# 7IBBE77S/nbodysim

Hardware: AMD Instinct MI355X
Metric: particle-pair interactions/sec at N=262,144 (direct O(N^2) softened gravity + kick/drift step) (higher is better)
Workload: dtype f32

## Files before the change

include/nbody.h:

```cpp
#ifndef NBODY_H
#define NBODY_H

#include <stddef.h>
#include <stdint.h>

#ifdef __cplusplus
extern "C" {
#endif
#pragma GCC visibility push(default)

#define NB_ABI_VERSION 8

typedef struct nb_vec2 {
    float x, y;
    float _pad[2];
} nb_vec2;

#define NB_Z(v) ((v)._pad[0])

typedef struct nb_body {
    nb_vec2 pos;
    nb_vec2 vel;
    nb_vec2 acc;
    float   mass;
// ... 328 lines not shown
    int64_t  r_base;
    uint32_t diag, group;
} nb_sym_item;

typedef struct nb_sym_info {
    uint32_t struct_size;
    int32_t  enabled;
    uint32_t chunks_per_item;
    uint32_t items, items_local, items_cross, items_late;
    uint32_t tiles, rows_s, segments, cus;
    uint64_t units_local, units_cross, units_late;
    uint64_t cross_units_total;
    uint64_t slab_s_bytes, slab_r_bytes;
    uint64_t coverage_entries;
    uint32_t tile_particles;
    uint32_t _reserved0;
} nb_sym_info;
int nb_sym_plan_info(const nb_sim *s, nb_sym_info *out);

int nb_device_count(void);

const char *nb_last_error(void);
int nb_last_error_code(void);

int nb_abi_version(void);

#pragma GCC visibility pop
#ifdef __cplusplus
}
#endif
#endif
// ... 1 lines not shown
```

nbodysim_amd/_lib.py:

```python
from __future__ import annotations

import ctypes as C
import os
from pathlib import Path

import numpy as np

PKG_DIR = Path(__file__).resolve().parent
LIB_PATH = PKG_DIR / "libnbody_hip.so"

NB_ABI_VERSION = 8

NB_OK, NB_EINVAL, NB_ENODEVICE, NB_EHIP, NB_ENOMEM, NB_EIO, NB_EFORMAT, NB_ESTATE = 0, -1, -2, -3, -4, -5, -6, -7
NB_FP32, NB_FP64 = 0, 1
NB_RSQRT_EXACT, NB_RSQRT_QUAKE = 0, 1
NB_SUM_TILED, NB_SUM_SEQUENTIAL = 0, 1
NB_EXTRA_VCLAMP, NB_EXTRA_BOUNDARY, NB_EXTRA_COLLIDE = 1, 2, 4
NB_INTEGRATOR_KICK_DRIFT, NB_INTEGRATOR_KDK, NB_INTEGRATOR_DKD, NB_INTEGRATOR_FR4 = 0, 1, 2, 3
NB_INTEGRATOR_HERMITE4 = 5
NB_FORCE_DIRECT, NB_FORCE_TREE = 0, 1
NB_POS_CURRENT, NB_POS_NEXT = 0, 1
NB_SHARD_NONE, NB_SHARD_ALLGATHER, NB_SHARD_SYMMETRIC, NB_SHARD_ALLREDUCE = 0, 1, 2, 3
NB_FLAG_NO_SYMMETRY, NB_FLAG_NO_UNIFORM_MASS, NB_FLAG_NO_GUIDED_TAIL, NB_FLAG_SHARD_ALLREDUCE, NB_FLAG_SHARD_SINGLE, NB_FLAG_MASS_SCALING = 1, 2, 4, 8, 16, 32
NB_FLAG_STATIC_ITEMS = 256
# ... 125 lines not shown
        ("items_local", C.c_uint32),
        ("items_cross", C.c_uint32),
        ("items_late", C.c_uint32),
        ("tiles", C.c_uint32),
        ("rows_s", C.c_uint32),
        ("segments", C.c_uint32),
        ("cus", C.c_uint32),
        ("units_local", C.c_uint64),
        ("units_cross", C.c_uint64),
        ("units_late", C.c_uint64),
        ("cross_units_total", C.c_uint64),
        ("slab_s_bytes", C.c_uint64),
        ("slab_r_bytes", C.c_uint64),
        ("coverage_entries", C.c_uint64),
        ("tile_particles", C.c_uint32),
        ("_reserved0", C.c_uint32),
    ]

    def as_dict(self) -> dict:
        return {k: int(getattr(self, k)) for k, _ in self._fields_ if k != "struct_size" and not k.startswith("_")}


class nb_view(C.Structure):

    _fields_ = [
        ("struct_size", C.c_uint32),
        ("width", C.c_uint32),
        ("height", C.c_uint32),
        ("center_x", C.c_float),
        ("center_y", C.c_float),
        ("scale", C.c_float),
# ... 206 lines not shown
```

nbodysim_amd/csrc/nb_capi.hip:

```cpp
#include "nb_sim.hip.h"

extern "C" int nb_device_count(void)
{
    int n = 0;
    if (hipGetDeviceCount(&n) != hipSuccess) { (void)hipGetLastError(); return 0; }
    return n;
}

static uint32_t even_slices(uint32_t jn, uint32_t want)
{
    const uint32_t tiles = (jn + TJ - 1) / TJ;
    if (want < 1) want = 1;
    if (want > tiles) want = tiles;
    const uint32_t per = (tiles + want - 1) / want;
    return (tiles + per - 1) / per;
}

static ForceJob plan_job(const nb_sim *s, uint32_t jb, uint32_t je, uint32_t slab0,
                         uint32_t gap_begin = 0xffffffffu, uint32_t gap_len = 0)
{
    ForceJob j{jb, je, 0, slab0, 1, 0, gap_begin, gap_len};
    const uint32_t ic = (uint32_t)s->i_count;
    if (je <= jb) return j;
    const uint32_t jn = je - jb;
// ... 120 lines not shown
static bool sym_uses_pairs(const nb_sim *s)
{
    if (!s->sym_pairs) return false;
    return s->dims3 ? s->uniform_mass || s->p.sym_chunk_pairs > 0 : !s->mass_scaled;
}

static SymTuning tuning_of(const nb_params &p, bool fp64, int cus, uint32_t world, bool sharded, size_t n)
{
    SymTuning t;
    t.forced_L = p.sym_chunks_per_item > 0 ? (uint32_t)p.sym_chunks_per_item : 0u;
    t.late_units = sharded ? late_units_for(p, fp64, cus, world) : 0u;
    t.wg_per_cu = sharded ? 24u : 0u;
    t.late_chunks = fp64 ? 1u : 2u;
    t.even_chunks = want_pairs(p, n);
    t.sb = sym_tile_of(p, n);
    t.guided_tail = !(p.flags & NB_FLAG_NO_GUIDED_TAIL);
    if (p.sym_tail[0] > 0.0f || p.sym_tail[1] > 0.0f || p.sym_tail[2] > 0.0f)
        { for (int k = 0; k < 3; ++k) t.tail_at[k] = (double)p.sym_tail[k]; t.tail_given = true; }
    return t;
}

static void fill_sym_info(const SymPlan &pl, uint32_t n, uint32_t world, int cus, size_t esz, bool enabled, nb_sym_info *out)
{
    const uint32_t sz = out->struct_size;
    memset(out, 0, sizeof *out);
    out->struct_size = sz;
    out->enabled = enabled ? 1 : 0;
    out->chunks_per_item = pl.L;
    out->items = (uint32_t)pl.items.size();
    out->items_local = pl.n_local; out->items_cross = pl.n_cross; out->items_late = pl.n_late;
    out->tiles = pl.tiles;
    out->rows_s = pl.rowbase.empty() ? 0u : pl.rowbase[pl.tiles];
    out->segments = (uint32_t)pl.segs.size();
    out->cus = (uint32_t)cus;
    out->units_local = pl.units_local; out->units_cross = pl.units_cross; out->units_late = pl.units_late;
    sym_units(n, world, nullptr, &out->cross_units_total, pl.sb);
    out->slab_s_bytes = (uint64_t)out->rows_s * pl.sb * esz;
    out->tile_particles = pl.sb;
    out->slab_r_bytes = pl.slab_r_elems * esz;
    out->coverage_entries = pl.cov_main.size() + pl.cov_late.size();
}

#ifdef NB_TEST_HOOKS
extern "C" int nb_debug_sym_plan(size_t n, int cus, int rank, int world, const nb_params *tuning,
                                 nb_sym_item *items_out, size_t cap, nb_sym_info *info)
{
    static_assert(sizeof(nb_sym_item) == sizeof(SymItem) && offsetof(nb_sym_item, r_base) == offsetof(SymItem, r_base) &&
                  offsetof(nb_sym_item, group) == offsetof(SymItem, group), "nb_sym_item mirrors SymItem");
    if (n == 0 || n > 0x7fffff00u || cus < 1 || world < 1 || rank < 0 || rank >= world ||
        (world > 1 && (n % ((size_t)world * SYM_SB)) != 0)) return nb_fail(NB_EINVAL, "nb_debug_sym_plan: bad arguments");
    if (tuning && tuning->struct_size != sizeof(nb_params)) return nb_fail(NB_EINVAL, "nb_debug_sym_plan: tuning->struct_size");
    if (info && info->struct_size != sizeof(nb_sym_info)) return nb_fail(NB_EINVAL, "nb_debug_sym_plan: info->struct_size");
    nb_params p;
    if (tuning) p = *tuning; else nb_params_default(&p);
    p.shard_rank = rank; p.shard_world = world;
// ... 114 lines not shown
    const uint32_t n = (uint32_t)s->n;
    const bool sharded = s->path == StepPath::SYM_SHARDED, split = s->path != StepPath::SYM;
    const uint32_t world = split ? (uint32_t)s->p.shard_world : 1u;
    const uint32_t rank = split ? (uint32_t)s->p.shard_rank : 0u;
    SymPlan pl;
    build_sym_plan(n, (uint32_t)s->cus, rank, world, tuning_of(s->p, s->fp64, s->cus, world, sharded, s->n), pl);
    s->sym_pairs = want_pairs(s->p, s->n);
    const uint32_t tiles = pl.tiles, row = pl.rowbase[tiles];
    s->sym_info.struct_size = (uint32_t)sizeof(nb_sym_info);
    fill_sym_info(pl, n, world, s->cus, s->esz, true, &s->sym_info);
    s->sym_items_local = pl.n_local; s->sym_items_cross = pl.n_cross; s->sym_items_late = pl.n_late;
    s->sym_items = (uint32_t)pl.items.size(); s->sym_tiles = tiles; s->sym_rows = row; s->sym_L = pl.L;
    s->sym_sb = pl.sb; s->sym_sb_shift = pl.sb == SYM_SB_WS ? 9u : 11u;
    std::vector<uint32_t> bounds(3 * (size_t)tiles);
    for (uint32_t g = 0; g < tiles; ++g) { bounds[g] = pl.rowbase[g]; bounds[tiles + g] = pl.rowmid[g]; bounds[2 * (size_t)tiles + g] = pl.rowbase[g + 1]; }
    std::vector<uint32_t> cbegin(pl.cov_main_begin);
    cbegin.insert(cbegin.end(), pl.cov_late_begin.begin(), pl.cov_late_begin.end());
    std::vector<SymCov> cov(pl.cov_main);
    cov.insert(cov.end(), pl.cov_late.begin(), pl.cov_late.end());
    s->sym_cov_late_off = (uint32_t)pl.cov_main.size();
    HIPCHK(s->pool.alloc(s->sym_items_dev, pl.items.size()));
    HIPCHK(s->pool.alloc(s->sym_rowbase_dev, bounds.size()));
    HIPCHK(s->pool.alloc(s->sym_cov_begin_dev, cbegin.size()));
    HIPCHK(s->pool.alloc(s->sym_cov_dev, cov.size() ? cov.size() : 1));
    HIPCHK(s->pool.alloc(s->sym_slab_s, (size_t)(row ? row : 1) * pl.sb * s->esz));
    HIPCHK(s->pool.alloc(s->sym_slab_r, (size_t)(pl.slab_r_elems ? pl.slab_r_elems : 1) * s->esz));
    int rc;
    if ((rc = copy_h2d(s, s->sym_items_dev, pl.items.data(), pl.items.size() * sizeof(SymItem)))) return rc;
    if ((rc = copy_h2d(s, s->sym_rowbase_dev, bounds.data(), bounds.size() * sizeof(uint32_t)))) return rc;
    if ((rc = copy_h2d(s, s->sym_cov_begin_dev, cbegin.data(), cbegin.size() * sizeof(uint32_t)))) return rc;
    if ((rc = copy_h2d(s, s->sym_cov_dev, cov.data(), cov.size() * sizeof(SymCov)))) return rc;
    HIPCHK(s->pool.alloc(s->sym_ticket, 3 * 128 / sizeof(uint32_t)));
    HIPCHK(hipMemsetAsync(s->sym_ticket, 0, 3 * 128, s->stream));
    s->aux_local = sharded && (s->p.sym_aux_stream ? s->p.sym_aux_stream > 0 : s->sym_items_local <= 4u * (uint32_t)s->cus);
    if (s->aux_local || s->sym_items_late) {
        HIPCHK(hipStreamCreateWithFlags(&s->aux, hipStreamNonBlocking));
        HIPCHK(hipEventCreateWithFlags(&s->ev_fork, hipEventDisableTiming));
        HIPCHK(hipEventCreateWithFlags(&s->ev_join, hipEventDisableTiming));
        HIPCHK(hipEventCreateWithFlags(&s->ev_late, hipEventDisableTiming));
    }
    if (split) {
// ... 1314 lines not shown
```

nbodysim_amd/csrc/nb_fuzz.cpp:

```cpp
#include <unistd.h>

#include <algorithm>
#include <cstdio>
#include <cstdlib>
#include <cstring>
#include <random>
#include <string>
#include <vector>

#include "nb_mem.h"
#include "nb_plan.h"
#include "nb_sched.h"
#include "nbody.h"

using namespace nbk;

#define REQUIRE(cond, ...)                                                        \
    do {                                                                          \
        if (!(cond)) {                                                            \
            std::fprintf(stderr, "FAIL %s:%d: %s | ", __FILE__, __LINE__, #cond); \
            std::fprintf(stderr, __VA_ARGS__);                                    \
            std::fprintf(stderr, "\n");                                           \
            std::exit(1);                                                         \
        }                                                                         \
    } while (0)

static void check_plan_case(uint32_t n, uint32_t world, uint32_t cus, const SymTuning &tune)
{
    const uint32_t sb = tune.sb;
    const uint32_t tiles = (n + sb - 1) / sb, chunks = (n + SYM_CH - 1) / SYM_CH, cpt = sb / SYM_CH;
    std::vector<uint8_t> cover((size_t)tiles * chunks, 0);
    uint64_t cross_seen = 0, cross_total = 0;
    sym_units(n, world, nullptr, &cross_total, sb);
    for (uint32_t rank = 0; rank < world; ++rank) {
        SymPlan pl;
        build_sym_plan(n, cus, rank, world, tune, pl);
        REQUIRE(pl.tiles == tiles && pl.sb == sb && pl.items.size() == (size_t)pl.n_local + pl.n_cross + pl.n_late, "n=%u world=%u", n, world);
        REQUIRE(pl.slab_r_elems <= sym_slab_r_bound(n, world, sb), "bound n=%u world=%u: %llu > %llu", n, world,
                (unsigned long long)pl.slab_r_elems, (unsigned long long)sym_slab_r_bound(n, world, sb));
        if (!tune.forced_L) REQUIRE(pl.L % tune.quantum() == 0, "L = %u is not a multiple of the kernel's chunk quantum %u", pl.L, tune.quantum());
        std::vector<uint8_t> row_used(pl.rowbase[tiles], 0);
        std::vector<std::pair<int64_t, int64_t>> ranges;
        for (const SymItem &it : pl.items) {
            REQUIRE(it.tile < tiles && it.cnt >= 1 && it.c0 + it.cnt <= chunks, "item out of range n=%u", n);
            REQUIRE(it.s_row < row_used.size() && !row_used[it.s_row], "stationary row reused n=%u", n);
            row_used[it.s_row] = 1;
            const uint32_t lo_row = it.group == 2 ? pl.rowmid[it.tile] : pl.rowbase[it.tile];
            const uint32_t hi_row = it.group == 2 ? pl.rowbase[it.tile + 1] : pl.rowmid[it.tile];
            REQUIRE(it.s_row >= lo_row && it.s_row < hi_row, "row outside its tile's range");
            if (it.diag) REQUIRE(it.c0 >= it.tile * cpt && it.c0 + it.cnt <= std::min((it.tile + 1) * cpt, chunks), "diag chunks");
            else {
                REQUIRE(it.c0 >= (it.tile + 1) * cpt, "symmetric item meets its own tile");
                const int64_t lo = it.r_base + (int64_t)it.c0 * SYM_CH;
                const int64_t hi = it.r_base + (int64_t)std::min<uint64_t>((uint64_t)(it.c0 + it.cnt) * SYM_CH, n);
                REQUIRE(lo >= 0 && hi <= (int64_t)pl.slab_r_elems && lo < hi, "travelling range outside the slab");
                ranges.push_back({lo, hi});
            }
            if (it.group == 1) cross_seen += it.cnt;
            for (uint32_t c = it.c0; c < it.c0 + it.cnt; ++c) {
                REQUIRE(cover[(size_t)it.tile * chunks + c] == 0, "unit (%u,%u) covered twice, n=%u world=%u", it.tile, c, n, world);
                cover[(size_t)it.tile * chunks + c] = 1;
            }
        }
        std::sort(ranges.begin(), ranges.end());
        int64_t end = 0;
        for (auto &r : ranges) { REQUIRE(r.first == end || r.first == end + 1, "travelling ranges overlap or leave a hole"); end = r.second; }
// ... 2 lines not shown
        auto check_cov = [&](size_t s0, size_t s1, const std::vector<uint32_t> &begin, const std::vector<SymCov> &cov) {
            REQUIRE(begin.size() == (size_t)tiles + 1 && begin[tiles] == cov.size(), "coverage CSR shape");
            uint64_t want = 0, got = 0;
            for (size_t s = s0; s < s1; ++s) want += pl.segs[s].hi - pl.segs[s].lo;
            for (uint32_t t = 0; t < tiles; ++t)
                for (uint32_t i = begin[t]; i < begin[t + 1]; ++i) {
                    const uint32_t a = std::max(cov[i].lo, t * sb), b = std::min<uint64_t>(cov[i].hi, (uint64_t)(t + 1) * sb);
                    REQUIRE(a < b, "coverage entry does not meet its tile");
                    REQUIRE(cov[i].base + (int64_t)a >= 0 && cov[i].base + (int64_t)b <= (int64_t)pl.slab_r_elems, "coverage outside the slab");
                    got += b - a;
                }
            REQUIRE(want == got, "coverage lists miss particles: %llu vs %llu", (unsigned long long)want, (unsigned long long)got);
        };
        check_cov(0, pl.nsegs_main, pl.cov_main_begin, pl.cov_main);
        check_cov(pl.nsegs_main, pl.segs.size(), pl.cov_late_begin, pl.cov_late);
    }
    for (uint32_t t = 0; t < tiles; ++t)
        for (uint32_t c = 0; c < chunks; ++c)
            REQUIRE(cover[(size_t)t * chunks + c] == (c >= t * cpt ? 1 : 0), "unit (%u,%u) cover %d, n=%u world=%u", t, c,
                    cover[(size_t)t * chunks + c], n, world);
    REQUIRE(cross_seen == cross_total, "cross units %llu != %llu", (unsigned long long)cross_seen, (unsigned long long)cross_total);
}

static void fuzz_planner(int cases, std::mt19937 &rng)
{
    for (int k = 0; k < cases; ++k) {
        const uint32_t world = 1 + rng() % 8;
        uint32_t n;
        if (world == 1) n = 1 + rng() % 200000;
        else n = world * SYM_SB * (2 + rng() % 12);
        const uint32_t cus = 1 + rng() % 304;
        SymTuning t;
        if (rng() % 3 == 0) t.forced_L = 1 + rng() % 70;
        if (world > 1 && rng() % 2) t.late_units = rng() % 3000;
        t.late_chunks = 1 + rng() % 3;
        t.guided_tail = rng() % 4 != 0;
        t.even_chunks = rng() % 2 != 0;
        if (rng() % 2) t.sb = SYM_SB_WS;
        if (rng() % 5 == 0) t.wg_per_cu = 8 + rng() % 32;
        if (rng() % 4 == 0) { t.tail_at[0] = 0.3; t.tail_at[1] = 0.6; t.tail_at[2] = 0.9; }
        check_plan_case(n, world, cus, t);
    }
    check_plan_case(262144, 8, 256, SymTuning{});
    { SymTuning e; e.even_chunks = true; e.late_units = 1400; check_plan_case(262144, 8, 256, e); check_plan_case(262144, 1, 256, e); check_plan_case(70001, 1, 256, e); }
    { SymTuning w; w.sb = SYM_SB_WS; check_plan_case(25000, 1, 256, w); check_plan_case(65536, 1, 256, w); check_plan_case(1, 1, 256, w); check_plan_case(513, 1, 2, w);
      w.even_chunks = true; check_plan_case(65536, 1, 256, w); check_plan_case(70001, 1, 256, w); check_plan_case(262144, 8, 256, w); }
    check_plan_case(1, 1, 256, SymTuning{});
    check_plan_case(2048, 1, 256, SymTuning{});
    check_plan_case(2049, 1, 1, SymTuning{});
}

static void write_raw(const std::string &path, const void *data, size_t bytes)
{
    FILE *f = std::fopen(path.c_str(), "wb");
    REQUIRE(f, "cannot create %s", path.c_str());
    REQUIRE(std::fwrite(data, 1, bytes, f) == bytes, "short write");
    std::fclose(f);
}

static void fuzz_host(const std::string &dir, std::mt19937 &rng)
{
    const std::string path = dir + "/fuzz.nbd";
    for (size_t n : {(size_t)1, (size_t)2, (size_t)4097, (size_t)10000}) {
        std::vector<nb_body> b(n), back(n);
// ... 258 lines not shown
```

nbodysim_amd/csrc/nb_kernels.hip.h:

```cpp
#pragma once
#include <hip/hip_runtime.h>
#include <stdint.h>
#include <type_traits>

#include "nb_plan.h"

namespace nbk {

typedef float v2f __attribute__((ext_vector_type(2)));
typedef float v4f __attribute__((ext_vector_type(4)));

constexpr int BLOCK = 256;
constexpr int TJ = 256;

enum { RSQ_EXACT = 0, RSQ_QUAKE = 1 };

constexpr float PAD_XY = 1.0e18f;

template <typename real> struct vec2_of;
template <> struct vec2_of<float> { typedef float2 type; };
template <> struct vec2_of<double> { typedef double2 type; };

template <typename real> struct vec4_of;
template <> struct vec4_of<float> { typedef float4 type; };
// ... 414 lines not shown
#define NB_SYM_UNROLL2 2
#endif
constexpr int SYM_P = NB_SYM_P;
constexpr int SYM_UNROLL = NB_SYM_UNROLL;
constexpr int SYM_UNROLL2 = NB_SYM_UNROLL2;
constexpr uint32_t SYM_WT = 64 * 2 * SYM_P;
static_assert(4 * SYM_WT == SYM_SB, "block-tile of the planner (nb_plan.h) = 4 waves x 64 lanes x 2 SYM_P particles");

__device__ __forceinline__ float lane_rot(float v, int addr)
{
    return __builtin_bit_cast(float, __builtin_amdgcn_ds_bpermute(addr, __builtin_bit_cast(int, v)));
}

enum { MM_UNIFORM = 0, MM_GENERAL = 1, MM_SCALED = 2 };

template <int RSQ, int MM, bool DIAG, bool WS = false, bool WT = false, typename L = Layout<float, false>>
__device__ __forceinline__
void sym_chunks(const typename L::vec *__restrict__ pos, const float *__restrict__ mass, const float *__restrict__ sigma,
                typename L::vec *__restrict__ slab_r_row, uint32_t n, uint32_t c0, uint32_t cnt,
                const v2f (&xi)[SYM_P], const v2f (&yi)[SYM_P], const v2f (&zi)[SYM_P], const v2f (&mi)[SYM_P],
                v2f (&ax)[SYM_P], v2f (&ay)[SYM_P], v2f (&az)[SYM_P], float eps2, float um_mass, typename L::vec (*red)[4][64])
{
    constexpr bool UM = MM == MM_UNIFORM, MS = MM == MM_SCALED;
    const uint32_t t = threadIdx.x, lane = t & 63u, w = t >> 6;
    const int addr = (int)(((lane + 1u) & 63u) * 4u);
    const v2f e2 = {eps2, eps2};

    float xq = PAD_XY, yq = PAD_XY, zq = PAD_XY, mq = MS ? -1.0f : 0.f, eq = eps2;
    auto fetch = [&](uint32_t j, float &x, float &y, float &z, float &m, float &e) {
        x = PAD_XY; y = PAD_XY; z = PAD_XY; m = MS ? -1.0f : 0.f; e = eps2;
        if (j < n) {
// ... 70 lines not shown
            if constexpr (L::dims3) zq = zr;
            if constexpr (!UM) mq = mr;
            if constexpr (MS) eq = er;
            if constexpr (!DIAG) {
                aqx.x = lane_rot(aqx.x, addr); aqx.y = lane_rot(aqx.y, addr);
                aqy.x = lane_rot(aqy.x, addr); aqy.y = lane_rot(aqy.y, addr);
                if constexpr (L::dims3) { aqz.x = lane_rot(aqz.x, addr); aqz.y = lane_rot(aqz.y, addr); }
            }
        }
        if constexpr (!DIAG) {
            typename L::vec r;
            if constexpr (L::dims3) r = make_float4(aqx.x + aqx.y, aqy.x + aqy.y, aqz.x + aqz.y, 0.f);
            else r = make_float2(aqx.x + aqx.y, aqy.x + aqy.y);
            if constexpr (UM) { r.x *= um_mass; r.y *= um_mass; if constexpr (L::dims3) r.z *= um_mass; }
            if constexpr (MS) { const float s2 = mq * mq; r.x *= s2; r.y *= s2; }
            if constexpr (WS) {
                const uint32_t j = (c0 + c) * SYM_CH + lane;
                if (j < n) store8<WT>(&slab_r_row[j], r);
            } else {
                typename L::vec (*rb)[64] = red[c & 1u];
                rb[w][lane] = r;
                __syncthreads();
                if (w == 0) {
                    const uint32_t j = (c0 + c) * SYM_CH + lane;
                    typename L::vec a = rb[0][lane];
#pragma unroll
                    for (int k = 1; k < 4; ++k) { a.x += rb[k][lane].x; a.y += rb[k][lane].y; if constexpr (L::dims3) a.z += rb[k][lane].z; }
                    if (j < n) { if constexpr (L::dims3) slab_r_row[j] = a; else store8<WT>(&slab_r_row[j], a); }
                }
            }
        }
        xq = xn; yq = yn;
        if constexpr (L::dims3) zq = zn;
        if constexpr (!UM) mq = mn;
        if constexpr (MS) eq = en;
    }
}

template <int RSQ, int MM, bool DIAG, bool WS = false, bool WT = false, typename L = Layout<float, false>>
__device__ __forceinline__
void sym_chunks2(const typename L::vec *__restrict__ pos, const float *__restrict__ mass,
                 typename L::vec *__restrict__ slab_r_row, uint32_t n, uint32_t c0, uint32_t cnt,
                 const v2f (&xi)[SYM_P], const v2f (&yi)[SYM_P], const v2f (&zi)[SYM_P], const v2f (&mi)[SYM_P],
                 v2f (&ax)[SYM_P], v2f (&ay)[SYM_P], v2f (&az)[SYM_P], float eps2, float um_mass, float4 (*red)[4][64])
{
    static_assert(MM != MM_SCALED, "the mass-scaled body keeps the one-chunk form");
    constexpr bool UM = MM == MM_UNIFORM;
    const uint32_t t = threadIdx.x, lane = t & 63u, w = t >> 6;
    const int addr = (int)(((lane + 1u) & 63u) * 4u);
    const v2f e2 = {eps2, eps2};
    v2f bx[2 * SYM_P], by[2 * SYM_P], bz[2 * SYM_P];
#pragma unroll
    for (int k = 0; k < 2 * SYM_P; ++k) { bx[k] = (v2f){0.f, 0.f}; by[k] = (v2f){0.f, 0.f}; bz[k] = (v2f){0.f, 0.f}; }

// ... 68 lines not shown
                    }
                }
            }
            xq = xr; yq = yr;
            if constexpr (L::dims3) zq = zr;
            if constexpr (!UM) mq = mr;
            if constexpr (!DIAG) {
                aqx = (v2f){lane_rot(aqx.x, addr), lane_rot(aqx.y, addr)};
                aqy = (v2f){lane_rot(aqy.x, addr), lane_rot(aqy.y, addr)};
                if constexpr (L::dims3) aqz = (v2f){lane_rot(aqz.x, addr), lane_rot(aqz.y, addr)};
            }
        }
        if constexpr (!DIAG && L::dims3) {
            float4 r0 = make_float4(aqx.x, aqy.x, aqz.x, 0.f), r1 = make_float4(aqx.y, aqy.y, aqz.y, 0.f);
            if constexpr (UM) { r0.x *= um_mass; r0.y *= um_mass; r0.z *= um_mass; r1.x *= um_mass; r1.y *= um_mass; r1.z *= um_mass; }
            float4 (*rb)[4][64] = red + 2u * ((c >> 1) & 1u);
            rb[0][w][lane] = r0;
            rb[1][w][lane] = r1;
            __syncthreads();
            if (w < 2 && c + w < cnt) {
                const uint32_t j = (c0 + c + w) * SYM_CH + lane;
                float4 a = rb[w][0][lane];
#pragma unroll
                for (int k = 1; k < 4; ++k) { a.x += rb[w][k][lane].x; a.y += rb[w][k][lane].y; a.z += rb[w][k][lane].z; }
                if (j < n) slab_r_row[j] = a;
            }
        } else if constexpr (!DIAG) {
            float4 r = make_float4(aqx.x, aqy.x, aqx.y, aqy.y);
            if constexpr (UM) { r.x *= um_mass; r.y *= um_mass; r.z *= um_mass; r.w *= um_mass; }
            if constexpr (WS) {
                const uint32_t j0 = (c0 + c) * SYM_CH + lane, j1 = j0 + SYM_CH;
                if (j0 < n) store8<WT>(&slab_r_row[j0], make_float2(r.x, r.y));
                if (c + 1 < cnt && j1 < n) store8<WT>(&slab_r_row[j1], make_float2(r.z, r.w));
            } else {
                float4 (*rb)[64] = red[(c >> 1) & 1u];
                rb[w][lane] = r;
                __syncthreads();
                if (w < 2 && c + w < cnt) {
                    const uint32_t j = (c0 + c + w) * SYM_CH + lane;
                    float2 a = w ? make_float2(rb[0][lane].z, rb[0][lane].w) : make_float2(rb[0][lane].x, rb[0][lane].y);
#pragma unroll
                    for (int k = 1; k < 4; ++k) {
                        a.x += w ? rb[k][lane].z : rb[k][lane].x;
                        a.y += w ? rb[k][lane].w : rb[k][lane].y;
                    }
// ... 46 lines not shown
            if (g0 < n) p0 = pos[g0];
            if (g1 < n) p1 = pos[g1];
            xi[p] = (v2f){p0.x, p1.x}; yi[p] = (v2f){p0.y, p1.y}; zi[p] = (v2f){p0.z, p1.z}; mi[p] = (v2f){p0.w, p1.w};
            az[p] = (v2f){0.f, 0.f};
        } else {
            float2 p0 = make_float2(PAD_XY, PAD_XY), p1 = p0;
            float m0 = 0.f, m1 = 0.f;
            if (g0 < n) { p0 = pos[g0]; if constexpr (!UM) m0 = mass[g0]; }
            if (g1 < n) { p1 = pos[g1]; if constexpr (!UM) m1 = mass[g1]; }
            xi[p] = (v2f){p0.x, p1.x}; yi[p] = (v2f){p0.y, p1.y}; mi[p] = (v2f){m0, m1};
        }
        ax[p] = (v2f){0.f, 0.f}; ay[p] = (v2f){0.f, 0.f};
    }
    NB_STAMP(1);
    typename L::vec *__restrict__ rrow = slab_r + it.r_base;
    if constexpr (PAIRS) {
        if (diag) sym_chunks2<RSQ, MM, true, WS, WT, L>(pos, mass, rrow, n, it.c0, it.cnt, xi, yi, zi, mi, ax, ay, az, eps2, um_mass, red2);
        else      sym_chunks2<RSQ, MM, false, WS, WT, L>(pos, mass, rrow, n, it.c0, it.cnt, xi, yi, zi, mi, ax, ay, az, eps2, um_mass, red2);
    } else {
        if (diag) sym_chunks<RSQ, MM, true, WS, WT, L>(pos, mass, sigma, rrow, n, it.c0, it.cnt, xi, yi, zi, mi, ax, ay, az, eps2, um_mass, red);
        else      sym_chunks<RSQ, MM, false, WS, WT, L>(pos, mass, sigma, rrow, n, it.c0, it.cnt, xi, yi, zi, mi, ax, ay, az, eps2, um_mass, red);
    }

    NB_STAMP(2);
    typename L::vec *__restrict__ out = slab_s + (size_t)s_row * SB;
    if constexpr (L::dims3) {
#pragma unroll
        for (int p = 0; p < SYM_P; ++p) {
            if constexpr (UM) { ax[p] *= um_mass; ay[p] *= um_mass; az[p] *= um_mass; }
            out[li[p]] = make_float4(ax[p].x, ay[p].x, az[p].x, 0.f);
            out[li[p] + 1] = make_float4(ax[p].y, ay[p].y, az[p].y, 0.f);
        }
    } else if constexpr (WS) {
#pragma unroll
        for (int p = 0; p < SYM_P; ++p) red4[w * SYM_P + p][lane] = make_float4(ax[p].x, ay[p].x, ax[p].y, ay[p].y);
        __syncthreads();
// ... 25 lines not shown

template <int RSQ, int MM, bool PAIRS = false, bool WS = false>
__global__ __launch_bounds__(BLOCK, NB_SYM_WAVES)
void force_sym_f32(const float2 *__restrict__ pos, const float *__restrict__ mass, const float *__restrict__ sigma,
                   const SymItem *__restrict__ items,
                   float2 *__restrict__ slab_s, float2 *__restrict__ slab_r,
                   uint32_t n, float eps2, float um_mass, uint32_t *ticket, uint32_t first_wave, uint32_t ticket_base)
{
#ifndef NB_SYM_WT
#define NB_SYM_WT true
#endif
    force_sym_f32_body<RSQ, MM, PAIRS, WS, NB_SYM_WT>(pos, mass, sigma, items[sym_item_index(ticket, first_wave, ticket_base)], slab_s, slab_r, n, eps2, um_mass);
}

template <int RSQ, bool UM, bool PAIRS = false>
__global__ __launch_bounds__(BLOCK, UM && !PAIRS ? 5 : 1)
void force_sym3_f32(const float4 *__restrict__ pos, const SymItem *__restrict__ items,
                    float4 *__restrict__ slab_s, float4 *__restrict__ slab_r, uint32_t n, float eps2, float um_mass,
                    uint32_t *ticket, uint32_t first_wave, uint32_t ticket_base)
{
    force_sym_f32_body<RSQ, UM ? MM_UNIFORM : MM_GENERAL, PAIRS, false, false, Layout<float, true>>(
        pos, nullptr, nullptr, items[sym_item_index(ticket, first_wave, ticket_base)], slab_s, slab_r, n, eps2, um_mass);
}

__global__ __launch_bounds__(BLOCK)
void mass_sigma(const float *__restrict__ mass, float *__restrict__ sigma, uint32_t n)
{
    const uint32_t i = blockIdx.x * BLOCK + threadIdx.x;
    if (i < n) sigma[i] = 1.0f / sqrtf(mass[i]);
}

// ... 709 lines not shown
```

nbodysim_amd/csrc/nb_plan.cpp:

```cpp
#include "nb_plan.h"

#include <cmath>

namespace nbk {

namespace {
struct Geometry {
    uint32_t n, world, sb, tiles, chunks, cpt, tpb;
    Geometry(uint32_t n_, uint32_t world_, uint32_t sb_) : n(n_), world(world_ ? world_ : 1), sb(sb_ ? sb_ : SYM_SB)
    {
        tiles = (n + sb - 1) / sb;
        chunks = (n + SYM_CH - 1) / SYM_CH;
        cpt = sb / SYM_CH;
        tpb = world > 1 ? (n / world) / sb : tiles;
        if (tpb == 0) tpb = 1;
    }
    uint32_t block_of(uint32_t I) const { return I / tpb; }
    uint32_t block_end_chunk(uint32_t I) const
    {
        const uint64_t e = (uint64_t)(I / tpb + 1) * tpb * cpt;
        return (world > 1 && e < chunks) ? (uint32_t)e : chunks;
    }
    uint32_t diag_end(uint32_t I) const { return (I + 1) * cpt < chunks ? (I + 1) * cpt : chunks; }
};
// ... 8 lines not shown
        const uint32_t be = g.block_end_chunk(I);
        const uint32_t b = g.world > 1 ? g.block_of(I) : 0;
        if (b < g.world) local_of[b] += be - g.diag_end(I);
        cross += g.chunks - be;
    }
    for (uint64_t v : local_of) if (v > local_max) local_max = v;
    if (local_sym_units) *local_sym_units = local_max;
    if (cross_total) *cross_total = cross;
}

uint64_t sym_slab_r_bound(uint32_t n, uint32_t world, uint32_t sb)
{
    uint64_t local = 0, cross = 0;
    sym_units(n, world, &local, &cross, sb);
    const uint64_t w = world ? world : 1;
    return (local + (cross + w - 1) / w + (uint64_t)(n / SYM_CH) + (sb ? sb : SYM_SB) / SYM_CH) * SYM_CH;
}

void build_sym_plan(uint32_t n, uint32_t cus, uint32_t rank, uint32_t world, const SymTuning &tune, SymPlan &pl)
{
    const Geometry g(n, world, tune.sb);
    world = g.world;
    const uint32_t tiles = g.tiles, chunks = g.chunks;
    if (cus < 1) cus = 1;

    uint64_t local = 0, cross_total = 0;
    for (uint32_t I = 0; I < tiles; ++I) {
        const uint32_t be = g.block_end_chunk(I);
        if (g.block_of(I) == rank || world == 1) local += be - I * g.cpt;
        cross_total += chunks - be;
    }
// ... 124 lines not shown
        next_cross[I] = row; row += cross_rows_of[I];
        pl.rowmid[I] = row;
        next_late[I] = row; row += late_rows_of[I];
        if (lhi[I] > llo[I]) add_seg(I, llo[I], lhi[I], 0u, base_local);
        if (chi[I] > clo[I]) add_seg(I, clo[I], chi[I], 1u, base_cross);
    }
    pl.rowbase[tiles] = row;
    pl.nsegs_main = (uint32_t)pl.segs.size();
    for (uint32_t I = 0; I < tiles; ++I)
        if (thi[I] > tlo[I]) add_seg(I, tlo[I], thi[I], 2u, base_late);
    pl.slab_r_elems = off;
    pl.units_local = pl.units_cross = pl.units_late = 0;
    for (auto &it : local_items) { it.s_row = next_local[it.tile]++; it.r_base = base_local[it.tile]; it.group = 0u; pl.units_local += it.cnt; }
    for (auto &it : cross_items) { it.s_row = next_cross[it.tile]++; it.r_base = base_cross[it.tile]; it.group = 1u; pl.units_cross += it.cnt; }
    for (auto &it : late_items)  { it.s_row = next_late[it.tile]++;  it.r_base = base_late[it.tile];  it.group = 2u; pl.units_late += it.cnt; }
    pl.n_local = (uint32_t)local_items.size();
    pl.n_cross = (uint32_t)cross_items.size();
    pl.n_late = (uint32_t)late_items.size();
    pl.items = std::move(local_items);
    pl.items.insert(pl.items.end(), cross_items.begin(), cross_items.end());
    pl.items.insert(pl.items.end(), late_items.begin(), late_items.end());
    pl.L = L;
    pl.tiles = tiles;
    pl.sb = g.sb;

    auto build_cov = [&](size_t s0, size_t s1, std::vector<uint32_t> &begin, std::vector<SymCov> &cov) {
        begin.assign((size_t)tiles + 1, 0);
        for (size_t s = s0; s < s1; ++s) {
            const SymSeg &sg = pl.segs[s];
            for (uint32_t t = sg.lo / g.sb; t <= (sg.hi - 1) / g.sb; ++t) ++begin[t + 1];
        }
        for (uint32_t t = 0; t < tiles; ++t) begin[t + 1] += begin[t];
        cov.assign(begin[tiles], SymCov{0, 0u, 0u});
        std::vector<uint32_t> fill(begin.begin(), begin.end() - 1);
        for (size_t s = s0; s < s1; ++s) {
            const SymSeg &sg = pl.segs[s];
            for (uint32_t t = sg.lo / g.sb; t <= (sg.hi - 1) / g.sb; ++t)
                cov[fill[t]++] = SymCov{(int64_t)sg.off - (int64_t)sg.lo, sg.lo, sg.hi};
        }
    };
    build_cov(0, pl.nsegs_main, pl.cov_main_begin, pl.cov_main);
    build_cov(pl.nsegs_main, pl.segs.size(), pl.cov_late_begin, pl.cov_late);
}

}
```

nbodysim_amd/csrc/nb_plan.h:

```cpp
#pragma once
#include <stdint.h>

#include <vector>

namespace nbk {

constexpr uint32_t SYM_SB = 2048;
constexpr uint32_t SYM_SB_WS = 512;
constexpr uint32_t SYM_WS_MAX_N = 49152;
constexpr uint32_t SYM_CH = 64;

struct SymItem { uint32_t tile, c0, cnt, s_row; int64_t r_base; uint32_t diag, group; };
static_assert(sizeof(SymItem) == 32, "SymItem is read by the kernels as 32 bytes");

struct SymSeg { uint32_t tile, lo, hi, group; uint64_t off; };

struct SymCov { int64_t base; uint32_t lo, hi; };
static_assert(sizeof(SymCov) == 16, "SymCov is read by the kernels as 16 bytes");

struct SymTuning {
    uint32_t forced_L = 0;
    uint32_t wg_per_cu = 0;
    uint32_t late_units = 0;
    uint32_t late_chunks = 2;
    bool guided_tail = true;
    bool even_chunks = false;
    uint32_t sb = SYM_SB;
    uint32_t quantum() const { return (sb == SYM_SB_WS ? 4u : 1u) * (even_chunks ? 2u : 1u); }
    double tail_at[3] = {0.85, 0.94, 0.98};
    bool tail_given = false;
};

struct SymPlan {
    std::vector<SymItem> items;
    uint32_t n_local = 0, n_cross = 0, n_late = 0, L = 0, tiles = 0, sb = SYM_SB;
    std::vector<uint32_t> rowbase, rowmid;
    std::vector<SymSeg> segs;
    uint32_t nsegs_main = 0;
    uint64_t slab_r_elems = 0;
    std::vector<uint32_t> cov_main_begin, cov_late_begin;
    std::vector<SymCov> cov_main, cov_late;
    uint64_t units_local = 0, units_cross = 0, units_late = 0;
};

void sym_units(uint32_t n, uint32_t world, uint64_t *local_sym_units, uint64_t *cross_total, uint32_t sb = SYM_SB);

uint64_t sym_slab_r_bound(uint32_t n, uint32_t world, uint32_t sb = SYM_SB);

void build_sym_plan(uint32_t n, uint32_t cus, uint32_t rank, uint32_t world, const SymTuning &tune, SymPlan &pl);

}
```

Measured before the change: 9938 billion.

## Exploit Newton's third law inside diagonal tiles using per-wave sub-block partials

Diagonal tiles of the symmetric force plan were previously computed as full all-pairs blocks. They are now split into four 512-particle sub-blocks per wave: each wave computes its own sub-block directly and a set of foreign sub-blocks symmetrically, writing the reaction partials to a new diagonal region of the receive slab. The coverage lists that later reduce the slab are merged with these diagonal entries per tile. This roughly halves diagonal-tile pair work at the cost of extra slab memory, more reduction traffic and a more complex plan. The launch bounds for the uniform-mass pairs kernel are also raised to request more waves per SIMD.

```diff
diff --git a/include/nbody.h b/include/nbody.h
--- a/include/nbody.h
+++ b/include/nbody.h
@@ -366,7 +366,7 @@
     uint64_t slab_s_bytes, slab_r_bytes;
     uint64_t coverage_entries;
     uint32_t tile_particles;
-    uint32_t _reserved0;
+    uint32_t diag_r_elems;
 } nb_sym_info;
 int nb_sym_plan_info(const nb_sim *s, nb_sym_info *out);
 
diff --git a/nbodysim_amd/_lib.py b/nbodysim_amd/_lib.py
--- a/nbodysim_amd/_lib.py
+++ b/nbodysim_amd/_lib.py
@@ -163,7 +163,7 @@
         ("slab_r_bytes", C.c_uint64),
         ("coverage_entries", C.c_uint64),
         ("tile_particles", C.c_uint32),
-        ("_reserved0", C.c_uint32),
+        ("diag_r_elems", C.c_uint32),
     ]
 
     def as_dict(self) -> dict:
diff --git a/nbodysim_amd/csrc/nb_capi.hip b/nbodysim_amd/csrc/nb_capi.hip
--- a/nbodysim_amd/csrc/nb_capi.hip
+++ b/nbodysim_amd/csrc/nb_capi.hip
@@ -158,6 +158,7 @@
     t.late_chunks = fp64 ? 1u : 2u;
     t.even_chunks = want_pairs(p, n);
     t.sb = sym_tile_of(p, n);
+    t.diag_sym = !fp64 && t.sb == SYM_SB;
     t.guided_tail = !(p.flags & NB_FLAG_NO_GUIDED_TAIL);
     if (p.sym_tail[0] > 0.0f || p.sym_tail[1] > 0.0f || p.sym_tail[2] > 0.0f)
         { for (int k = 0; k < 3; ++k) t.tail_at[k] = (double)p.sym_tail[k]; t.tail_given = true; }
@@ -183,6 +184,7 @@
     out->tile_particles = pl.sb;
     out->slab_r_bytes = pl.slab_r_elems * esz;
     out->coverage_entries = pl.cov_main.size() + pl.cov_late.size();
+    out->diag_r_elems = (uint32_t)pl.slab_d_elems;
 }
 
 #ifdef NB_TEST_HOOKS
@@ -327,17 +329,26 @@
     s->sym_sb = pl.sb; s->sym_sb_shift = pl.sb == SYM_SB_WS ? 9u : 11u;
     std::vector<uint32_t> bounds(3 * (size_t)tiles);
     for (uint32_t g = 0; g < tiles; ++g) { bounds[g] = pl.rowbase[g]; bounds[tiles + g] = pl.rowmid[g]; bounds[2 * (size_t)tiles + g] = pl.rowbase[g + 1]; }
-    std::vector<uint32_t> cbegin(pl.cov_main_begin);
-    cbegin.insert(cbegin.end(), pl.cov_late_begin.begin(), pl.cov_late_begin.end());
-    std::vector<SymCov> cov(pl.cov_main);
-    cov.insert(cov.end(), pl.cov_late.begin(), pl.cov_late.end());
-    s->sym_cov_late_off = (uint32_t)pl.cov_main.size();
+    std::vector<uint32_t> cbegin;
+    std::vector<SymCov> cov;
+    auto merged = [&](const std::vector<uint32_t> &b, const std::vector<SymCov> &c, const std::vector<uint32_t> &db, const std::vector<SymCov> &dc) {
+        const uint32_t first = (uint32_t)cov.size();
+        for (uint32_t g = 0; g < tiles; ++g) {
+            cbegin.push_back((uint32_t)cov.size() - first);
+            cov.insert(cov.end(), c.begin() + b[g], c.begin() + b[g + 1]);
+            cov.insert(cov.end(), dc.begin() + db[g], dc.begin() + db[g + 1]);
+        }
+        cbegin.push_back((uint32_t)cov.size() - first);
+    };
+    merged(pl.cov_main_begin, pl.cov_main, pl.dcov_main_begin, pl.dcov_main);
+    s->sym_cov_late_off = (uint32_t)cov.size();
+    merged(pl.cov_late_begin, pl.cov_late, pl.dcov_late_begin, pl.dcov_late);
     HIPCHK(s->pool.alloc(s->sym_items_dev, pl.items.size()));
     HIPCHK(s->pool.alloc(s->sym_rowbase_dev, bounds.size()));
     HIPCHK(s->pool.alloc(s->sym_cov_begin_dev, cbegin.size()));
     HIPCHK(s->pool.alloc(s->sym_cov_dev, cov.size() ? cov.size() : 1));
     HIPCHK(s->pool.alloc(s->sym_slab_s, (size_t)(row ? row : 1) * pl.sb * s->esz));
-    HIPCHK(s->pool.alloc(s->sym_slab_r, (size_t)(pl.slab_r_elems ? pl.slab_r_elems : 1) * s->esz));
+    HIPCHK(s->pool.alloc(s->sym_slab_r, (size_t)(pl.slab_r_alloc_elems() ? pl.slab_r_alloc_elems() : 1) * s->esz));
     int rc;
     if ((rc = copy_h2d(s, s->sym_items_dev, pl.items.data(), pl.items.size() * sizeof(SymItem)))) return rc;
     if ((rc = copy_h2d(s, s->sym_rowbase_dev, bounds.data(), bounds.size() * sizeof(uint32_t)))) return rc;
diff --git a/nbodysim_amd/csrc/nb_fuzz.cpp b/nbodysim_amd/csrc/nb_fuzz.cpp
--- a/nbodysim_amd/csrc/nb_fuzz.cpp
+++ b/nbodysim_amd/csrc/nb_fuzz.cpp
@@ -1,6 +1,7 @@
 #include <unistd.h>
 
 #include <algorithm>
+#include <map>
 #include <cstdio>
 #include <cstdlib>
 #include <cstring>
@@ -31,13 +32,18 @@
     const uint32_t tiles = (n + sb - 1) / sb, chunks = (n + SYM_CH - 1) / SYM_CH, cpt = sb / SYM_CH;
     std::vector<uint8_t> cover((size_t)tiles * chunks, 0);
     uint64_t cross_seen = 0, cross_total = 0;
+    std::map<uint32_t, std::vector<uint8_t>> diag_met;
     sym_units(n, world, nullptr, &cross_total, sb);
     for (uint32_t rank = 0; rank < world; ++rank) {
         SymPlan pl;
         build_sym_plan(n, cus, rank, world, tune, pl);
         REQUIRE(pl.tiles == tiles && pl.sb == sb && pl.items.size() == (size_t)pl.n_local + pl.n_cross + pl.n_late, "n=%u world=%u", n, world);
-        REQUIRE(pl.slab_r_elems <= sym_slab_r_bound(n, world, sb), "bound n=%u world=%u: %llu > %llu", n, world,
-                (unsigned long long)pl.slab_r_elems, (unsigned long long)sym_slab_r_bound(n, world, sb));
+        REQUIRE(pl.slab_r_alloc_elems() <= sym_slab_r_bound(n, world, sb), "bound n=%u world=%u: %llu > %llu", n, world,
+                (unsigned long long)pl.slab_r_alloc_elems(), (unsigned long long)sym_slab_r_bound(n, world, sb));
+        const bool dsym = tune.diag_sym && sb == SYM_SB;
+        const uint64_t d0 = (pl.slab_r_elems + 1u) & ~(uint64_t)1;
+        REQUIRE(dsym || (pl.slab_d_elems == 0 && pl.dsegs.empty() && pl.dcov_main.empty() && pl.dcov_late.empty()), "diagonal partials in a plan without them");
+        std::vector<uint8_t> dmark(pl.slab_d_elems, 0);
         if (!tune.forced_L) REQUIRE(pl.L % tune.quantum() == 0, "L = %u is not a multiple of the kernel's chunk quantum %u", pl.L, tune.quantum());
         std::vector<uint8_t> row_used(pl.rowbase[tiles], 0);
         std::vector<std::pair<int64_t, int64_t>> ranges;
@@ -48,8 +54,30 @@
             const uint32_t lo_row = it.group == 2 ? pl.rowmid[it.tile] : pl.rowbase[it.tile];
             const uint32_t hi_row = it.group == 2 ? pl.rowbase[it.tile + 1] : pl.rowmid[it.tile];
             REQUIRE(it.s_row >= lo_row && it.s_row < hi_row, "row outside its tile's range");
-            if (it.diag) REQUIRE(it.c0 >= it.tile * cpt && it.c0 + it.cnt <= std::min((it.tile + 1) * cpt, chunks), "diag chunks");
-            else {
+            if (it.diag) {
+                REQUIRE(it.c0 >= it.tile * cpt && it.c0 + it.cnt <= std::min((it.tile + 1) * cpt, chunks), "diag chunks");
+                if (dsym) {
+                    const uint32_t t0 = it.tile * cpt;
+                    std::vector<uint8_t> &met = diag_met[it.tile];
+                    if (met.empty()) met.assign((size_t)cpt * cpt, 0);
+                    for (uint32_t c = it.c0; c < it.c0 + it.cnt; ++c) {
+                        const uint32_t rel = c - t0, sub = rel / SYM_SUB_CH;
+                        for (uint32_t s = 0; s < SYM_SUB_CH; ++s) ++met[(size_t)(sub * SYM_SUB_CH + s) * cpt + rel];
+                        for (uint32_t w = 0; w < 4; ++w)
+                            for (uint32_t f = 0; f < sym_diag_foreign_count(w); ++f) {
+                                if (sym_diag_foreign(w, f) != sub) continue;
+                                for (uint32_t s = 0; s < SYM_SUB_CH; ++s) {
+                                    ++met[(size_t)(w * SYM_SUB_CH + s) * cpt + rel];
+                                    ++met[(size_t)rel * cpt + w * SYM_SUB_CH + s];
+                                }
+                                const int64_t lo = it.r_base + (f ? SYM_DIAG_ROW_B : 0) + (int64_t)c * SYM_CH;
+                                const int64_t hi = it.r_base + (f ? SYM_DIAG_ROW_B : 0) + (int64_t)std::min<uint64_t>((uint64_t)(c + 1) * SYM_CH, n);
+                                REQUIRE(lo >= (int64_t)d0 && hi <= (int64_t)pl.slab_r_alloc_elems() && lo < hi, "diagonal partial outside its part of the slab");
+                                for (int64_t e = lo; e < hi; ++e) { REQUIRE(dmark[e - d0] == 0, "diagonal partial written twice"); dmark[e - d0] = 1; }
+                            }
+                    }
+                }
+            } else {
                 REQUIRE(it.c0 >= (it.tile + 1) * cpt, "symmetric item meets its own tile");
                 const int64_t lo = it.r_base + (int64_t)it.c0 * SYM_CH;
                 const int64_t hi = it.r_base + (int64_t)std::min<uint64_t>((uint64_t)(it.c0 + it.cnt) * SYM_CH, n);
@@ -82,7 +110,29 @@
         };
         check_cov(0, pl.nsegs_main, pl.cov_main_begin, pl.cov_main);
         check_cov(pl.nsegs_main, pl.segs.size(), pl.cov_late_begin, pl.cov_late);
-    }
+        for (const auto *lists : {&pl.dcov_main, &pl.dcov_late}) {
+            const std::vector<uint32_t> &begin = lists == &pl.dcov_main ? pl.dcov_main_begin : pl.dcov_late_begin;
+            REQUIRE(begin.size() == (size_t)tiles + 1 && begin[tiles] == lists->size(), "diagonal coverage CSR shape");
+            for (uint32_t t = 0; t < tiles; ++t)
+                for (uint32_t i = begin[t]; i < begin[t + 1]; ++i) {
+                    const SymCov &cv = (*lists)[i];
+                    REQUIRE(cv.lo < cv.hi && cv.lo >= t * sb && cv.hi <= std::min<uint64_t>((uint64_t)(t + 1) * sb, n) && cv.lo % SYM_CH == 0 && cv.base % 2 == 0, "diagonal coverage entry outside its tile");
+                    for (uint32_t k = cv.lo; k < cv.hi; ++k) {
+                        const int64_t e = cv.base + (int64_t)k - (int64_t)d0;
+                        REQUIRE(e >= 0 && e < (int64_t)dmark.size() && dmark[e] == 1, "diagonal coverage reads what no item wrote, or reads it twice");
+                        dmark[e] = 3;
+                    }
+                }
+        }
+        for (uint8_t m : dmark) REQUIRE(m == 0 || m == 3, "a diagonal partial is written and never read");
+    }
+    for (const auto &tm : diag_met) {
+        const uint32_t t0 = tm.first * cpt, have = std::min((tm.first + 1) * cpt, chunks) - t0;
+        for (uint32_t a = 0; a < have; ++a)
+            for (uint32_t b = 0; b < have; ++b)
+                REQUIRE(tm.second[(size_t)a * cpt + b] == 1, "tile %u: chunk %u meets chunk %u %d times, n=%u world=%u", tm.first, a, b, tm.second[(size_t)a * cpt + b], n, world);
+    }
+    if (tune.diag_sym && sb == SYM_SB) REQUIRE(diag_met.size() == tiles, "a tile without diagonal items");
     for (uint32_t t = 0; t < tiles; ++t)
         for (uint32_t c = 0; c < chunks; ++c)
             REQUIRE(cover[(size_t)t * chunks + c] == (c >= t * cpt ? 1 : 0), "unit (%u,%u) cover %d, n=%u world=%u", t, c,
@@ -105,6 +155,7 @@
         t.guided_tail = rng() % 4 != 0;
         t.even_chunks = rng() % 2 != 0;
         if (rng() % 2) t.sb = SYM_SB_WS;
+        else t.diag_sym = rng() % 4 != 0;
         if (rng() % 5 == 0) t.wg_per_cu = 8 + rng() % 32;
         if (rng() % 4 == 0) { t.tail_at[0] = 0.3; t.tail_at[1] = 0.6; t.tail_at[2] = 0.9; }
         check_plan_case(n, world, cus, t);
@@ -116,6 +167,10 @@
     check_plan_case(1, 1, 256, SymTuning{});
     check_plan_case(2048, 1, 256, SymTuning{});
     check_plan_case(2049, 1, 1, SymTuning{});
+    { SymTuning d; d.diag_sym = true;
+      for (uint32_t n : {1u, 63u, 1024u, 1025u, 1100u, 2048u, 2118u, 6143u, 70001u}) { check_plan_case(n, 1, 256, d); d.even_chunks = !d.even_chunks; }
+      d.forced_L = 3; check_plan_case(6143, 1, 256, d); d.forced_L = 5; d.even_chunks = true; check_plan_case(2118, 1, 256, d); d.forced_L = 0;
+      d.even_chunks = true; check_plan_case(262144, 1, 256, d); d.late_units = 1400; check_plan_case(262144, 8, 256, d); check_plan_case(131072, 4, 256, d); }
 }
 
 static void write_raw(const std::string &path, const void *data, size_t bytes)
diff --git a/nbodysim_amd/csrc/nb_kernels.hip.h b/nbodysim_amd/csrc/nb_kernels.hip.h
--- a/nbodysim_amd/csrc/nb_kernels.hip.h
+++ b/nbodysim_amd/csrc/nb_kernels.hip.h
@@ -452,7 +452,7 @@
 
 enum { MM_UNIFORM = 0, MM_GENERAL = 1, MM_SCALED = 2 };
 
-template <int RSQ, int MM, bool DIAG, bool WS = false, bool WT = false, typename L = Layout<float, false>>
+template <int RSQ, int MM, bool DIAG, bool WS = false, bool WT = false, typename L = Layout<float, false>, bool SOLO = false>
 __device__ __forceinline__
 void sym_chunks(const typename L::vec *__restrict__ pos, const float *__restrict__ mass, const float *__restrict__ sigma,
                 typename L::vec *__restrict__ slab_r_row, uint32_t n, uint32_t c0, uint32_t cnt,
@@ -553,9 +553,9 @@
             else r = make_float2(aqx.x + aqx.y, aqy.x + aqy.y);
             if constexpr (UM) { r.x *= um_mass; r.y *= um_mass; if constexpr (L::dims3) r.z *= um_mass; }
             if constexpr (MS) { const float s2 = mq * mq; r.x *= s2; r.y *= s2; }
-            if constexpr (WS) {
+            if constexpr (WS || SOLO) {
                 const uint32_t j = (c0 + c) * SYM_CH + lane;
-                if (j < n) store8<WT>(&slab_r_row[j], r);
+                if (j < n) { if constexpr (L::dims3) slab_r_row[j] = r; else store8<WT>(&slab_r_row[j], r); }
             } else {
                 typename L::vec (*rb)[64] = red[c & 1u];
                 rb[w][lane] = r;
@@ -576,7 +576,7 @@
     }
 }
 
-template <int RSQ, int MM, bool DIAG, bool WS = false, bool WT = false, typename L = Layout<float, false>>
+template <int RSQ, int MM, bool DIAG, bool WS = false, bool WT = false, typename L = Layout<float, false>, bool SOLO = false>
 __device__ __forceinline__
 void sym_chunks2(const typename L::vec *__restrict__ pos, const float *__restrict__ mass,
                  typename L::vec *__restrict__ slab_r_row, uint32_t n, uint32_t c0, uint32_t cnt,
@@ -675,6 +675,11 @@
         if constexpr (!DIAG && L::dims3) {
             float4 r0 = make_float4(aqx.x, aqy.x, aqz.x, 0.f), r1 = make_float4(aqx.y, aqy.y, aqz.y, 0.f);
             if constexpr (UM) { r0.x *= um_mass; r0.y *= um_mass; r0.z *= um_mass; r1.x *= um_mass; r1.y *= um_mass; r1.z *= um_mass; }
+            if constexpr (SOLO) {
+                const uint32_t j0 = (c0 + c) * SYM_CH + lane, j1 = j0 + SYM_CH;
+                if (j0 < n) slab_r_row[j0] = r0;
+                if (c + 1 < cnt && j1 < n) slab_r_row[j1] = r1;
+            } else {
             float4 (*rb)[4][64] = red + 2u * ((c >> 1) & 1u);
             rb[0][w][lane] = r0;
             rb[1][w][lane] = r1;
@@ -686,10 +691,11 @@
                 for (int k = 1; k < 4; ++k) { a.x += rb[w][k][lane].x; a.y += rb[w][k][lane].y; a.z += rb[w][k][lane].z; }
                 if (j < n) slab_r_row[j] = a;
             }
+            }
         } else if constexpr (!DIAG) {
             float4 r = make_float4(aqx.x, aqy.x, aqx.y, aqy.y);
             if constexpr (UM) { r.x *= um_mass; r.y *= um_mass; r.z *= um_mass; r.w *= um_mass; }
-            if constexpr (WS) {
+            if constexpr (WS || SOLO) {
                 const uint32_t j0 = (c0 + c) * SYM_CH + lane, j1 = j0 + SYM_CH;
                 if (j0 < n) store8<WT>(&slab_r_row[j0], make_float2(r.x, r.y));
                 if (c + 1 < cnt && j1 < n) store8<WT>(&slab_r_row[j1], make_float2(r.z, r.w));
@@ -766,12 +772,37 @@
     }
     NB_STAMP(1);
     typename L::vec *__restrict__ rrow = slab_r + it.r_base;
-    if constexpr (PAIRS) {
-        if (diag) sym_chunks2<RSQ, MM, true, WS, WT, L>(pos, mass, rrow, n, it.c0, it.cnt, xi, yi, zi, mi, ax, ay, az, eps2, um_mass, red2);
-        else      sym_chunks2<RSQ, MM, false, WS, WT, L>(pos, mass, rrow, n, it.c0, it.cnt, xi, yi, zi, mi, ax, ay, az, eps2, um_mass, red2);
-    } else {
-        if (diag) sym_chunks<RSQ, MM, true, WS, WT, L>(pos, mass, sigma, rrow, n, it.c0, it.cnt, xi, yi, zi, mi, ax, ay, az, eps2, um_mass, red);
-        else      sym_chunks<RSQ, MM, false, WS, WT, L>(pos, mass, sigma, rrow, n, it.c0, it.cnt, xi, yi, zi, mi, ax, ay, az, eps2, um_mass, red);
+    auto sweep = [&](auto dg, auto solo, typename L::vec *__restrict__ row, uint32_t c0, uint32_t cnt) {
+        constexpr bool DG = decltype(dg)::value, SO = decltype(solo)::value;
+        if constexpr (PAIRS) sym_chunks2<RSQ, MM, DG, WS, WT, L, SO>(pos, mass, row, n, c0, cnt, xi, yi, zi, mi, ax, ay, az, eps2, um_mass, red2);
+        else sym_chunks<RSQ, MM, DG, WS, WT, L, SO>(pos, mass, sigma, row, n, c0, cnt, xi, yi, zi, mi, ax, ay, az, eps2, um_mass, red);
+    };
+    using yes = std::integral_constant<bool, true>;
+    using no = std::integral_constant<bool, false>;
+    if constexpr (WS) {
+        if constexpr (PAIRS) {
+            if (diag) sym_chunks2<RSQ, MM, true, WS, WT, L>(pos, mass, rrow, n, it.c0, it.cnt, xi, yi, zi, mi, ax, ay, az, eps2, um_mass, red2);
+            else      sym_chunks2<RSQ, MM, false, WS, WT, L>(pos, mass, rrow, n, it.c0, it.cnt, xi, yi, zi, mi, ax, ay, az, eps2, um_mass, red2);
+        } else {
+            if (diag) sym_chunks<RSQ, MM, true, WS, WT, L>(pos, mass, sigma, rrow, n, it.c0, it.cnt, xi, yi, zi, mi, ax, ay, az, eps2, um_mass, red);
+            else      sym_chunks<RSQ, MM, false, WS, WT, L>(pos, mass, sigma, rrow, n, it.c0, it.cnt, xi, yi, zi, mi, ax, ay, az, eps2, um_mass, red);
+        }
+    } else if (!diag) sweep(no{}, no{}, rrow, it.c0, it.cnt);
+    else {
+        const uint32_t wu = (uint32_t)__builtin_amdgcn_readfirstlane((int)w);
+        const uint32_t t0 = it.tile * (SYM_SB / SYM_CH), i1 = it.c0 + it.cnt;
+        auto clip = [&](uint32_t sub, uint32_t &lo) {
+            const uint32_t a = t0 + sub * SYM_SUB_CH, b = a + SYM_SUB_CH;
+            lo = it.c0 > a ? it.c0 : a;
+            const uint32_t hi = i1 < b ? i1 : b;
+            return hi > lo ? hi - lo : 0u;
+        };
+        uint32_t lo, cn = clip(wu, lo);
+        if (cn) sweep(yes{}, no{}, rrow, lo, cn);
+        for (uint32_t f = 0; f < sym_diag_foreign_count(wu); ++f) {
+            cn = clip(sym_diag_foreign(wu, f), lo);
+            if (cn) sweep(no{}, yes{}, rrow + (f ? SYM_DIAG_ROW_B : 0u), lo, cn);
+        }
     }
 
     NB_STAMP(2);
@@ -827,7 +858,7 @@
 }
 
 template <int RSQ, bool UM, bool PAIRS = false>
-__global__ __launch_bounds__(BLOCK, UM && !PAIRS ? 5 : 1)
+__global__ __launch_bounds__(BLOCK, UM ? (PAIRS ? 3 : 5) : 1)
 void force_sym3_f32(const float4 *__restrict__ pos, const SymItem *__restrict__ items,
                     float4 *__restrict__ slab_s, float4 *__restrict__ slab_r, uint32_t n, float eps2, float um_mass,
                     uint32_t *ticket, uint32_t first_wave, uint32_t ticket_base)
diff --git a/nbodysim_amd/csrc/nb_plan.cpp b/nbodysim_amd/csrc/nb_plan.cpp
--- a/nbodysim_amd/csrc/nb_plan.cpp
+++ b/nbodysim_amd/csrc/nb_plan.cpp
@@ -46,7 +46,8 @@
     uint64_t local = 0, cross = 0;
     sym_units(n, world, &local, &cross, sb);
     const uint64_t w = world ? world : 1;
-    return (local + (cross + w - 1) / w + (uint64_t)(n / SYM_CH) + (sb ? sb : SYM_SB) / SYM_CH) * SYM_CH;
+    const uint64_t tiles = ((uint64_t)n + SYM_SB - 1) / SYM_SB;
+    return (local + (cross + w - 1) / w + (uint64_t)(n / SYM_CH) + (sb ? sb : SYM_SB) / SYM_CH) * SYM_CH + tiles * (2 * SYM_SB + 4) + 2;
 }
 
 void build_sym_plan(uint32_t n, uint32_t cus, uint32_t rank, uint32_t world, const SymTuning &tune, SymPlan &pl)
@@ -201,6 +202,36 @@
     for (auto &it : local_items) { it.s_row = next_local[it.tile]++; it.r_base = base_local[it.tile]; it.group = 0u; pl.units_local += it.cnt; }
     for (auto &it : cross_items) { it.s_row = next_cross[it.tile]++; it.r_base = base_cross[it.tile]; it.group = 1u; pl.units_cross += it.cnt; }
     for (auto &it : late_items)  { it.s_row = next_late[it.tile]++;  it.r_base = base_late[it.tile];  it.group = 2u; pl.units_late += it.cnt; }
+    pl.dsegs.clear();
+    uint64_t doff = (off + 1u) & ~(uint64_t)1;
+    const uint64_t dstart = doff;
+    auto diag_segs = [&](std::vector<SymItem> &list, uint32_t group) {
+        std::vector<uint32_t> lo(tiles, 0xffffffffu), hi(tiles, 0);
+        for (const auto &it : list) {
+            if (!it.diag) continue;
+            if (it.c0 < lo[it.tile]) lo[it.tile] = it.c0;
+            if (it.c0 + it.cnt > hi[it.tile]) hi[it.tile] = it.c0 + it.cnt;
+        }
+        std::vector<int64_t> base(tiles, 0);
+        for (uint32_t I = 0; I < tiles; ++I) {
+            if (hi[I] <= lo[I]) continue;
+            const uint32_t plo = up((uint64_t)lo[I] * SYM_CH, n), phi = up((uint64_t)hi[I] * SYM_CH, n), mid = I * g.sb + SYM_DIAG_ROW_B;
+            base[I] = (int64_t)doff - (int64_t)plo;
+            pl.dsegs.push_back(SymSeg{I, plo, phi, group, doff});
+            uint64_t len = phi - plo;
+            if (phi > mid) {
+                const uint32_t blo = plo > mid ? plo : mid;
+                pl.dsegs.push_back(SymSeg{I, blo, phi, group, doff + (blo - plo) + SYM_DIAG_ROW_B});
+                len += SYM_DIAG_ROW_B;
+            }
+            doff += (len + 1u) & ~(uint64_t)1;
+        }
+        for (auto &it : list) if (it.diag) it.r_base = base[it.tile];
+    };
+    if (tune.diag_sym && g.sb == SYM_SB) diag_segs(local_items, 0u);
+    pl.ndsegs_main = (uint32_t)pl.dsegs.size();
+    if (tune.diag_sym && g.sb == SYM_SB) diag_segs(late_items, 2u);
+    pl.slab_d_elems = doff - dstart;
     pl.n_local = (uint32_t)local_items.size();
     pl.n_cross = (uint32_t)cross_items.size();
     pl.n_late = (uint32_t)late_items.size();
@@ -211,23 +242,25 @@
     pl.tiles = tiles;
     pl.sb = g.sb;
 
-    auto build_cov = [&](size_t s0, size_t s1, std::vector<uint32_t> &begin, std::vector<SymCov> &cov) {
+    auto build_cov = [&](const std::vector<SymSeg> &segs, size_t s0, size_t s1, std::vector<uint32_t> &begin, std::vector<SymCov> &cov) {
         begin.assign((size_t)tiles + 1, 0);
         for (size_t s = s0; s < s1; ++s) {
-            const SymSeg &sg = pl.segs[s];
+            const SymSeg &sg = segs[s];
             for (uint32_t t = sg.lo / g.sb; t <= (sg.hi - 1) / g.sb; ++t) ++begin[t + 1];
         }
         for (uint32_t t = 0; t < tiles; ++t) begin[t + 1] += begin[t];
         cov.assign(begin[tiles], SymCov{0, 0u, 0u});
         std::vector<uint32_t> fill(begin.begin(), begin.end() - 1);
         for (size_t s = s0; s < s1; ++s) {
-            const SymSeg &sg = pl.segs[s];
+            const SymSeg &sg = segs[s];
             for (uint32_t t = sg.lo / g.sb; t <= (sg.hi - 1) / g.sb; ++t)
                 cov[fill[t]++] = SymCov{(int64_t)sg.off - (int64_t)sg.lo, sg.lo, sg.hi};
         }
     };
-    build_cov(0, pl.nsegs_main, pl.cov_main_begin, pl.cov_main);
-    build_cov(pl.nsegs_main, pl.segs.size(), pl.cov_late_begin, pl.cov_late);
-}
-
-}
+    build_cov(pl.segs, 0, pl.nsegs_main, pl.cov_main_begin, pl.cov_main);
+    build_cov(pl.segs, pl.nsegs_main, pl.segs.size(), pl.cov_late_begin, pl.cov_late);
+    build_cov(pl.dsegs, 0, pl.ndsegs_main, pl.dcov_main_begin, pl.dcov_main);
+    build_cov(pl.dsegs, pl.ndsegs_main, pl.dsegs.size(), pl.dcov_late_begin, pl.dcov_late);
+}
+
+}
diff --git a/nbodysim_amd/csrc/nb_plan.h b/nbodysim_amd/csrc/nb_plan.h
--- a/nbodysim_amd/csrc/nb_plan.h
+++ b/nbodysim_amd/csrc/nb_plan.h
@@ -12,6 +12,10 @@
 
 struct SymItem { uint32_t tile, c0, cnt, s_row; int64_t r_base; uint32_t diag, group; };
 static_assert(sizeof(SymItem) == 32, "SymItem is read by the kernels as 32 bytes");
+
+constexpr uint32_t SYM_SUB = 512, SYM_SUB_CH = 8, SYM_DIAG_ROW_B = 1024;
+constexpr uint32_t sym_diag_foreign_count(uint32_t w) { return w < 2u ? 2u : 1u; }
+constexpr uint32_t sym_diag_foreign(uint32_t w, uint32_t f) { return f == 0u ? ((w + 1u) & 3u) : w + 2u; }
 
 struct SymSeg { uint32_t tile, lo, hi, group; uint64_t off; };
 
@@ -29,6 +33,7 @@
     uint32_t quantum() const { return (sb == SYM_SB_WS ? 4u : 1u) * (even_chunks ? 2u : 1u); }
     double tail_at[3] = {0.85, 0.94, 0.98};
     bool tail_given = false;
+    bool diag_sym = false;
 };
 
 struct SymPlan {
@@ -41,6 +46,12 @@
     std::vector<uint32_t> cov_main_begin, cov_late_begin;
     std::vector<SymCov> cov_main, cov_late;
     uint64_t units_local = 0, units_cross = 0, units_late = 0;
+    std::vector<SymSeg> dsegs;
+    uint32_t ndsegs_main = 0;
+    uint64_t slab_d_elems = 0;
+    std::vector<uint32_t> dcov_main_begin, dcov_late_begin;
+    std::vector<SymCov> dcov_main, dcov_late;
+    uint64_t slab_r_alloc_elems() const { return ((slab_r_elems + 1u) & ~(uint64_t)1) + slab_d_elems; }
 };
 
 void sym_units(uint32_t n, uint32_t world, uint64_t *local_sym_units, uint64_t *cross_total, uint32_t sb = SYM_SB);
```

After: 9943 billion (median of 2 runs). About the same (+0.1%).
